# lazear/sage

Hardware: AMD Instinct MI355X
Metric: spectra/sec (whole node), fragment-index search-and-score, human tryptic narrow search (higher is better)
Workload: dtype f32

## Files before the change

### include/sage_hip.h

```cpp
#ifndef SAGE_HIP_H
#define SAGE_HIP_H

#include <stddef.h>
#include <stdint.h>

#ifdef __cplusplus
extern "C" {
#endif

#define SAGE_HIP_ABI_VERSION 6

enum {
    SAGE_HIP_OK = 0,
    SAGE_HIP_ERR_INVALID = 1,
    SAGE_HIP_ERR_NO_DEVICE = 2,
    SAGE_HIP_ERR_HIP = 3,
    SAGE_HIP_ERR_UNSUPPORTED = 4,
    SAGE_HIP_ERR_OOM = 5,
    SAGE_HIP_ERR_INTERNAL = 6
};

enum { SAGE_TOL_PPM = 0, SAGE_TOL_PCT = 1, SAGE_TOL_DA = 2 };
typedef struct SageTolerance {
    int32_t kind;
// ... 160 lines not shown
    uint64_t capacity;
    uint64_t* psm_off;
    uint8_t* kinds;
    int32_t* charges;
    int32_t* fragment_ordinals;
    float* intensities;
    float* mz_calculated;
    float* mz_experimental;
} SageFragments;
int sage_hip_annotate_resident(SageScorer* scorer, SageDeviceBatch* batch, const SageFeature* features,
                               const uint32_t* counts, SageFragments* out);

int sage_hip_quick_score_resident(SageScorer* scorer, SageDeviceBatch* batch, int prefilter_low_memory, uint8_t* keep);

typedef struct SageTiming {
    float prelim_ms;
    float rescore_ms;
    float total_ms;
    uint32_t n_launches;
    uint32_t n_wide;
    uint32_t arena_entries;
    uint32_t n_retry;
    float retry_ms;
    uint32_t n_tied;
    uint32_t n_ways;
} SageTiming;
int sage_hip_last_timing(const SageScorer* scorer, SageTiming* out);
int sage_hip_scorer_set_timing_interval(SageScorer* scorer, uint32_t every);

int sage_hip_host_alloc(uint64_t bytes, void** out);
void sage_hip_host_free(void* p);

int sage_hip_debug_phase_cycles(SageScorer* scorer, unsigned long long* out32);

typedef struct SageRescoreInput {
    uint64_t n;
    const SageFeature* features;
    const float* aligned_rt;
    const float* delta_rt_model;
    const float* delta_ims_model;
    SageTolerance precursor_tol;
    const uint32_t* peptide_key;
    uint32_t n_peptide_keys;
    const uint32_t* protein_key;
    uint32_t n_protein_keys;
} SageRescoreInput;

typedef struct SageRescoreOutput {
    float* discriminant_score;
    float* posterior_error;
    float* spectrum_q;
    float* peptide_q;
    float* protein_q;
    uint32_t* order;
    uint64_t passing_spectrum;
    uint64_t passing_peptide;
    uint64_t passing_protein;
    int32_t lda_fitted;
    double coef[20];
    float device_ms;
} SageRescoreOutput;

int sage_hip_rescore(int device, const SageRescoreInput* in, SageRescoreOutput* out);

typedef struct SageRtInput {
    uint64_t n;
// ... 168 lines not shown
```

### sage_amd/_lib.py

```python
import ctypes as C
import os

import numpy as np

from . import build as _build

c_float_p = C.POINTER(C.c_float)
c_u8_p = C.POINTER(C.c_uint8)
c_u32_p = C.POINTER(C.c_uint32)
c_u64_p = C.POINTER(C.c_uint64)


class SageTolerance(C.Structure):
    _fields_ = [("kind", C.c_int32), ("lo", C.c_float), ("hi", C.c_float)]


class SageTheoretical(C.Structure):
    _fields_ = [("peptide_index", C.c_uint32), ("fragment_mz", C.c_float)]


class SageDbParams(C.Structure):
    _fields_ = [
        ("bucket_size", C.c_uint64),
        ("missed_cleavages", C.c_int32),
# ... 241 lines not shown
        "sage_hip_abi_version": (C.c_int, []),
        "sage_hip_hostdb_build": (C.c_int, [C.c_char_p, C.POINTER(SageDbParams), C.POINTER(vp)]),
        "sage_hip_hostdb_free": (None, [vp]),
        "sage_hip_hostdb_view": (C.c_int, [vp, C.POINTER(SageDbView)]),
        "sage_hip_hostdb_peptide_string": (C.c_uint64, [vp, C.c_uint64, C.c_char_p, C.c_uint64]),
        "sage_hip_hostdb_peptide_proteins": (C.c_uint64, [vp, C.c_uint64, C.c_char_p, C.c_uint64]),
        "sage_hip_hostdb_peptide_info": (C.c_int, [vp, C.c_uint64, c_u32_p, c_u8_p]),
        "sage_hip_process_ms2": (C.c_uint64, [C.c_uint64, C.c_int, C.c_float, c_float_p, c_float_p, C.c_uint64,
                                              C.c_uint8, c_float_p, c_float_p, c_float_p]),
        "sage_hip_device_count": (C.c_int, []),
        "sage_hip_db_create": (C.c_int, [C.POINTER(SageDbView), C.c_int, C.POINTER(vp)]),
        "sage_hip_db_destroy": (None, [vp]),
        "sage_hip_db_device_bytes": (C.c_uint64, [vp]),
        "sage_hip_scorer_create": (C.c_int, [vp, C.POINTER(SageScorerParams), C.POINTER(vp)]),
        "sage_hip_scorer_destroy": (None, [vp]),
        "sage_hip_scorer_clone": (C.c_int, [vp, C.POINTER(vp)]),
        "sage_hip_score_batch": (C.c_int, [vp, C.POINTER(SageSpectrumBatch), vp, c_u32_p]),
        "sage_hip_batch_upload": (C.c_int, [vp, C.POINTER(SageSpectrumBatch), C.POINTER(vp)]),
        "sage_hip_batch_free": (None, [vp]),
        "sage_hip_batch_process_upload": (C.c_int, [vp, C.POINTER(SageRawBatch), C.c_uint64, C.c_int, C.c_float, C.c_uint32,
                                                    C.POINTER(vp), c_u32_p]),
        "sage_hip_batch_download": (C.c_int, [vp, c_u64_p, c_float_p, c_float_p, c_float_p]),
        "sage_hip_batch_upload_kinds": (C.c_int, [vp, C.POINTER(SageSpectrumBatch), c_u8_p, C.POINTER(vp)]),
        "sage_hip_batch_process_upload_kinds": (C.c_int, [vp, C.POINTER(SageRawBatch), c_u8_p, C.c_uint64, C.c_int, C.c_float,
                                                          C.c_uint32, C.POINTER(vp), c_u32_p]),
        "sage_hip_score_batch_kinds": (C.c_int, [vp, C.POINTER(SageSpectrumBatch), c_u8_p, vp, c_u32_p]),
        "sage_hip_score_resident": (C.c_int, [vp, vp, vp, c_u32_p]),
        "sage_hip_initial_hits": (C.c_int, [vp, vp, c_u64_p, C.c_uint32, c_u32_p, c_u64_p, c_u64_p]),
        "sage_hip_last_timing": (C.c_int, [vp, C.POINTER(SageTiming)]),
        "sage_hip_scorer_set_timing_interval": (C.c_int, [vp, C.c_uint32]),
        "sage_hip_annotate_resident": (C.c_int, [vp, vp, vp, c_u32_p, C.POINTER(SageFragments)]),
        "sage_hip_quick_score_resident": (C.c_int, [vp, vp, C.c_int, c_u8_p]),
        "sage_hip_debug_phase_cycles": (C.c_int, [vp, c_u64_p]),
        "sage_hip_host_alloc": (C.c_int, [C.c_uint64, C.POINTER(vp)]),
        "sage_hip_host_free": (None, [vp]),
        "sage_hip_rescore": (C.c_int, [C.c_int, C.POINTER(SageRescoreInput), C.POINTER(SageRescoreOutput)]),
        "sage_hip_hostdb_competition_keys": (C.c_int, [vp, c_u32_p, C.c_uint64, c_u32_p, c_u32_p, c_u32_p, c_u32_p]),
        "sage_hip_predict_rt": (C.c_int, [C.c_int, C.POINTER(SageRtInput), C.POINTER(SageRtOutput)]),
        "sage_hip_hostdb_feature_peptides": (C.c_int, [vp, c_u32_p, C.c_uint64, c_u64_p, c_u8_p, c_float_p]),
        "sage_hip_mzml_read": (C.c_int, [C.c_char_p, C.c_uint32, C.c_int, C.POINTER(vp)]),
        "sage_hip_mzml_view": (C.c_int, [vp, C.POINTER(SageRawBatch)]),
        "sage_hip_mzml_check_searchable": (C.c_int, [vp]),
        "sage_hip_mzml_spectrum_id": (C.c_char_p, [vp, C.c_uint64]),
        "sage_hip_mzml_free": (None, [vp]),
        "sage_hip_mzml_read_sn": (C.c_int, [C.c_char_p, C.c_uint32, C.c_int, C.c_int, C.POINTER(vp)]),
        "sage_hip_mzml_ion_injection_time": (C.c_float, [vp, C.c_uint64]),
        "sage_hip_mzml_precursor_ref": (C.c_char_p, [vp, C.c_uint64]),
        "sage_hip_mgf_read": (C.c_int, [C.c_char_p, C.c_uint32, C.POINTER(vp)]),
        "sage_hip_mzml_isolation_kinds": (C.c_int, [vp, c_u8_p]),
        "sage_hip_mzml_charge_zero": (C.c_int, [vp, c_u8_p]),
        "sage_hip_parse_f32": (C.c_int, [C.c_char_p, C.c_uint64, c_float_p]),
        "sage_hip_tmt": (C.c_int, [C.c_int, C.POINTER(SageTmtInput), C.POINTER(SageTmtOutput)]),
        "sage_hip_write_tmt": (C.c_int, [C.c_char_p, C.POINTER(C.c_char_p), C.c_uint32, C.c_uint64, c_u32_p, C.POINTER(C.c_char_p),
                                         c_float_p, c_float_p, C.POINTER(C.c_char_p), C.c_uint32]),
        "sage_hip_write_results": (C.c_int, [C.c_char_p, C.c_int, vp, vp, C.c_uint64, c_u64_p, c_u64_p, C.POINTER(C.c_char_p),
                                             C.c_uint32, C.POINTER(C.c_char_p), C.POINTER(SagePostColumns)]),
        "sage_hip_lfq": (C.c_int, [C.c_int, C.POINTER(SageLfqInput), C.POINTER(SageLfqOutput)]),
        "sage_hip_lfq_im": (C.c_int, [C.c_int, C.POINTER(SageLfqInput), C.POINTER(SageLfqMobility), C.POINTER(SageLfqOutput)]),
        "sage_hip_mzml_mobility": (c_float_p, [vp]),
        "sage_hip_mzml_has_mobility": (C.c_int, [vp, c_u8_p]),
        "sage_hip_write_lfq": (C.c_int, [C.c_char_p, vp, C.POINTER(SageLfqOutput), c_u64_p, C.c_uint64, C.POINTER(C.c_char_p),
                                         C.c_uint32]),
        "sage_hip_fasta_num_targets": (C.c_int, [C.c_char_p, C.POINTER(SageDbParams), c_u64_p]),
        "sage_hip_prefilter_chunk_size": (C.c_int, [C.c_char_p, C.POINTER(SageDbParams), C.c_uint64, c_u64_p]),
        "sage_hip_hostdb_build_chunk": (C.c_int, [C.c_char_p, C.POINTER(SageDbParams), C.c_uint64, C.c_uint64, C.POINTER(vp)]),
        "sage_hip_hostdb_merge_kept": (C.c_int, [C.POINTER(vp), C.POINTER(c_u8_p), C.c_uint32, C.POINTER(SageDbParams),
                                                 C.POINTER(vp)]),
    }
    for name, (res, args) in sig.items():
        fn = getattr(lib, name)
        fn.restype = res
        fn.argtypes = args
    _lib = lib
    return lib


EXPORTED_SYMBOLS = [
    "sage_hip_last_error", "sage_hip_abi_version", "sage_hip_hostdb_build", "sage_hip_hostdb_free",
    "sage_hip_hostdb_view", "sage_hip_hostdb_peptide_string", "sage_hip_hostdb_peptide_proteins",
    "sage_hip_hostdb_peptide_info", "sage_hip_process_ms2", "sage_hip_device_count", "sage_hip_db_create", "sage_hip_db_destroy",
    "sage_hip_db_device_bytes", "sage_hip_scorer_create", "sage_hip_scorer_destroy", "sage_hip_scorer_clone", "sage_hip_score_batch",
    "sage_hip_batch_upload", "sage_hip_batch_free", "sage_hip_batch_process_upload", "sage_hip_batch_download", "sage_hip_score_resident", "sage_hip_initial_hits",
    "sage_hip_last_timing", "sage_hip_scorer_set_timing_interval", "sage_hip_annotate_resident", "sage_hip_quick_score_resident", "sage_hip_debug_phase_cycles", "sage_hip_host_alloc", "sage_hip_host_free",
    "sage_hip_rescore", "sage_hip_hostdb_competition_keys", "sage_hip_fasta_num_targets", "sage_hip_prefilter_chunk_size",
    "sage_hip_hostdb_build_chunk", "sage_hip_hostdb_merge_kept", "sage_hip_predict_rt", "sage_hip_hostdb_feature_peptides",
    "sage_hip_write_results", "sage_hip_mzml_read", "sage_hip_mzml_view", "sage_hip_mzml_check_searchable", "sage_hip_mzml_spectrum_id", "sage_hip_mzml_free",
    "sage_hip_lfq", "sage_hip_write_lfq", "sage_hip_mzml_read_sn", "sage_hip_mzml_ion_injection_time", "sage_hip_mzml_precursor_ref",
    "sage_hip_tmt", "sage_hip_write_tmt", "sage_hip_mgf_read", "sage_hip_mzml_isolation_kinds", "sage_hip_mzml_charge_zero",
    "sage_hip_parse_f32", "sage_hip_batch_upload_kinds", "sage_hip_batch_process_upload_kinds", "sage_hip_score_batch_kinds",
    "sage_hip_lfq_im", "sage_hip_mzml_mobility", "sage_hip_mzml_has_mobility",
]


def check(rc):
    if rc != 0:
        msg = load().sage_hip_last_error()
        raise SageHipError(f"libsage_hip status {rc}: {msg.decode() if msg else ''}")


def as_ptr(arr, ctype):
    return arr.ctypes.data_as(C.POINTER(ctype))
```

### sage_amd/csrc/capi.hip

```cpp
#include <hip/hip_runtime.h>
#include <algorithm>
#include <atomic>
#include <cmath>
#include <chrono>
#include <cstring>
#include <memory>
#include <future>
#include <mutex>
#include <string>
#include <vector>

#include "crlog.h"
#include "device_types.h"
#define HIP_FAILED(e, what) fail(status_of(e), std::string(what) + ": " + hipGetErrorString(e))
#include "hip_host.h"
#include "host_db.hpp"

using namespace sagehip;

namespace {

thread_local std::string g_last_error;

int fail(int code, const std::string& msg) {
// ... 721 lines not shown
            const double a = std::fabs((double)b);
            ok = ok && a > 0.0 && (double)ion_lo / 255.0 * a >= 2.0 * lo && (double)ion_hi * a <= 0.5 * hi;
        }
    if (ok) mode |= sagecore::TOL_FAST;
    return mode;
}

static int scorer_init(SageScorer* sp, SageDeviceDb* db, const SageScorerParams* p) {
    SageScorer* s = sp;
    s->db = db;
    s->params = *p;
    DevScorer& d = s->dev;
    d.precursor_tol = {p->precursor_tol.kind, p->precursor_tol.lo, p->precursor_tol.hi};
    d.fragment_tol = {p->fragment_tol.kind, p->fragment_tol.lo, p->fragment_tol.hi};
    d.pbm_reach = sagecore::pbm_reach_of(d.fragment_tol);
    d.min_matched_peaks = p->min_matched_peaks;
    d.min_isotope_err = p->min_isotope_err;
    d.max_isotope_err = p->max_isotope_err;
    d.min_precursor_charge = p->min_precursor_charge;
    d.max_precursor_charge = p->max_precursor_charge;
    d.override_precursor_charge = p->override_precursor_charge;
    d.max_fragment_charge = p->max_fragment_charge;
    d.chimera = p->chimera;
    d.report_psms = p->report_psms;
    d.wide_window = p->wide_window;
    d.score_type = p->score_type;
    d.kmax = std::max<uint32_t>(50, 2 * p->report_psms);
    const uint32_t n_iso = (uint32_t)(p->max_isotope_err - p->min_isotope_err) + 1;
    const uint32_t n_z = (uint32_t)(p->max_precursor_charge - p->min_precursor_charge) + 1;
    d.list_cap = d.kmax * (std::max(n_iso, n_z) + 1);
    d.wcap = 1024;
    d.dbg_flags = 0;
    if (const char* e = getenv("SAGE_HIP_DEBUG_FLAGS")) d.dbg_flags = (uint32_t)atoi(e);
    d.rescore_general = 0;
    if (const char* e = getenv("SAGE_HIP_RESCORE_GENERAL")) d.rescore_general = atoi(e) != 0 ? 1u : 0u;
    d.exact = 0;
    d.xcd_chunk = 1024;
    if (const char* e = getenv("SAGE_HIP_XCD_CHUNK")) d.xcd_chunk = (uint32_t)std::max(0, atoi(e));
    {
        const char* e = getenv("SAGE_HIP_SCHED_DESC");
        if (!e || atoi(e)) d.xcd_chunk |= 0x80000000u;
        s->sched_desc_forced = e != nullptr;
    }
    if (const char* e = getenv("SAGE_HIP_EXACT")) s->exact_always = atoi(e) != 0;
    if (const char* e = getenv("SAGE_HIP_FUSED")) s->fused = atoi(e) != 0;
    if (const char* e = getenv("SAGE_HIP_ONE_LANE")) s->two_lanes = atoi(e) == 0;
    if (const char* e = getenv("SAGE_HIP_SEARCH_LAG")) s->search_lag = (uint32_t)std::max(0, atoi(e));
    if (const char* e = getenv("SAGE_HIP_REPLAY_WAVE_MAX")) s->replay_split = (uint64_t)atoll(e) & 0xFFFFFFFFull;
    if (const char* e = getenv("SAGE_HIP_REPLAY_LANE_MAX")) s->replay_split |= (uint64_t)(uint32_t)atoll(e) << 32;
    if (const char* e = getenv("SAGE_HIP_ONE_LAUNCH")) s->one_launch = atoi(e) != 0;
#ifndef SAGE_HIP_EXPERIMENTS
    if (s->one_launch || s->fused || getenv("SAGE_HIP_SEARCH_LAG"))
        return fail(SAGE_HIP_ERR_UNSUPPORTED, "SAGE_HIP_ONE_LAUNCH / SAGE_HIP_FUSED / SAGE_HIP_SEARCH_LAG need a build with -DSAGE_HIP_EXPERIMENTS");
#endif
    if (const char* e = getenv("SAGE_HIP_NO_ZEROCOPY")) s->zero_copy = atoi(e) == 0;
    if (const char* e = getenv("SAGE_HIP_NO_FAST_TIES")) s->fast_ties = atoi(e) == 0;
    if (const char* e = getenv("SAGE_HIP_WCAP")) d.wcap = (uint32_t)std::min(16384, std::max(64, atoi(e)));
    if (const char* e = getenv("SAGE_HIP_CHUNK")) s->chunk = (uint32_t)std::min(1 << 22, std::max(64, atoi(e)));
    HIP_TRY(hipStreamCreateWithFlags(&s->stream, hipStreamNonBlocking));
    HIP_TRY(hipStreamCreateWithFlags(&s->up_stream, hipStreamNonBlocking));
    HIP_TRY(hipStreamCreateWithFlags(&s->down_stream, hipStreamNonBlocking));
    HIP_TRY(hipStreamCreateWithFlags(&s->side_stream, hipStreamNonBlocking));
    if (const char* e = getenv("SAGE_HIP_WAYS")) s->ways = (uint32_t)std::min(4, std::max(1, atoi(e)));
    if (p->report_psms != 1 || p->chimera) s->fast_ties = false;
    if ((d.wcap + 1) / 2 > fast_tie_lds_words()) s->fast_ties = false;
    s->cnt_stride = 4u + (((d.wcap + 1) / 2 + 3u) & ~3u);
// ... 21 lines not shown
        HIP_TRY(o.down_done.create(false));
        HIP_TRY(o.counters.alloc(2 * CTR_COUNT));
        HIP_TRY(hipHostMalloc((void**)&o.h_counters, 2 * CTR_COUNT * 4, hipHostMallocDefault));
        HIP_TRY(hipHostGetDevicePointer((void**)&o.h_counters_view, o.h_counters, 0));
    }
    for (SageDeviceBatch& b : s->slots) {
        b.device = db->device;
        HIP_TRY(b.up_done.create(false));
    }
    std::vector<double> tbl(131072);
    tbl[0] = 1.0;
    for (uint32_t n = 1; n < tbl.size(); n++) {
        const double x = (double)n;
        tbl[n] = x * sagecore::cr_log(x) - x + 0.5 * sagecore::cr_log(x) + 0.5 * sagecore::cr_log(M_PI * 2.0 * x);
    }
    HIP_TRY(s->lnfact.upload(tbl.data(), tbl.size()));
    {
        hipDeviceProp_t prop;
        HIP_TRY(hipGetDeviceProperties(&prop, db->device));
        const size_t tile_lds = ((size_t)1 << db->view.tile_shift) * 2 + 12 * 1024;
        const uint32_t per_cu = (uint32_t)std::max<size_t>(1, std::min<size_t>(4, (160 * 1024) / tile_lds));
        s->tile_blocks = (uint32_t)prop.multiProcessorCount * per_cu;
        const size_t tile_lds8 = ((size_t)1 << db->view.tile_shift) + 14 * 1024;
        s->tile_blocks8 = (uint32_t)prop.multiProcessorCount * (uint32_t)std::max<size_t>(1, std::min<size_t>(4, (160 * 1024) / tile_lds8));
        if (const char* e = getenv("SAGE_HIP_TILE_BLOCKS")) s->tile_blocks = s->tile_blocks8 = (uint32_t)std::max(1, atoi(e));
        if (const char* e = getenv("SAGE_HIP_NO_U8")) s->cnt8 = atoi(e) == 0;
        if (const char* e = getenv("SAGE_HIP_NO_REUSE")) s->reuse_counts = atoi(e) == 0;
        HIP_TRY((hipError_t)tile_kernel_prepare(160 * 1024));
        HIP_TRY((hipError_t)spectrum_kernel_prepare(160 * 1024));
    }
    s->qmax = queries_per_spectrum(d);
    if (const char* e = getenv("SAGE_HIP_PHASE_CLOCKS")) {
        if (atoi(e) > 0) {
            HIP_TRY(s->dbg.alloc(4096 * 32));
            HIP_TRY(hipMemset(s->dbg.p, 0, 4096 * 32 * 8));
        }
    }
    return SAGE_HIP_OK;
}

static void scorer_release(SageScorer* s) {
    (void)hipSetDevice(s->db->device);
    for (hipStream_t st : {s->stream, s->up_stream, s->down_stream, s->side_stream, s->way_stream[0], s->way_stream[1], s->way_stream[2]})
        if (st) {
            (void)hipStreamSynchronize(st);
            (void)hipStreamDestroy(st);
        }
    delete s;
}

int sage_hip_scorer_create(SageDeviceDb* db, const SageScorerParams* p, SageScorer** out) {
    if (!db || !p || !out) return fail(SAGE_HIP_ERR_INVALID, "null argument");
    if (p->report_psms == 0) return fail(SAGE_HIP_ERR_INVALID, "report_psms must be >= 1");
    if (p->report_psms > 32767) return fail(SAGE_HIP_ERR_UNSUPPORTED, "report_psms > 32767");
    if (p->min_isotope_err > p->max_isotope_err) return fail(SAGE_HIP_ERR_INVALID, "min_isotope_err > max_isotope_err");
    if (p->min_precursor_charge > p->max_precursor_charge || p->min_precursor_charge == 0)
        return fail(SAGE_HIP_ERR_INVALID, "precursor charge range must be [lo >= 1, hi >= lo]");
    if (p->score_type != 0 && p->score_type != 1) return fail(SAGE_HIP_ERR_INVALID, "unknown score_type");
    HIP_TRY(hipSetDevice(db->device));
    SageScorer* s = new SageScorer();
    const int rc = scorer_init(s, db, p);
    if (rc != SAGE_HIP_OK) {
        s->db = db;
        scorer_release(s);
        return rc;
    }
    *out = s;
    return SAGE_HIP_OK;
// ... 1136 lines not shown
    int rc = enqueue_compute(s, b->view, o, false, MODE_EXACT, s->stream);
    if (rc != SAGE_HIP_OK) return rc;
    HIP_TRY(hipMemcpyAsync(o.h_counters, o.counters.p, 2 * CTR_COUNT * 4, hipMemcpyDeviceToHost, s->stream));
    HIP_TRY(hipStreamSynchronize(s->stream));
    rc = collect(s, o, nullptr);
    if (rc != SAGE_HIP_OK) return rc;
    const uint32_t n = b->n, kmax = s->dev.kmax;
    std::vector<uint64_t> c((size_t)n * kmax);
    std::vector<uint32_t> tot((size_t)n * 2), st(n);
    HIP_TRY(hipMemcpy(c.data(), s->ws.cand.p, c.size() * 8, hipMemcpyDeviceToHost));
    HIP_TRY(hipMemcpy(len, s->ws.cand_len.p, (size_t)n * 4, hipMemcpyDeviceToHost));
    HIP_TRY(hipMemcpy(tot.data(), s->ws.totals.p, tot.size() * 4, hipMemcpyDeviceToHost));
    HIP_TRY(hipMemcpy(st.data(), s->ws.status.p, (size_t)n * 4, hipMemcpyDeviceToHost));
    for (uint32_t i = 0; i < n; i++) {
        if (st[i] != ST_OK && st[i] != ST_OK_ORDERED) return fail(SAGE_HIP_ERR_UNSUPPORTED, "spectrum " + std::to_string(i) + ": status " + std::to_string(st[i]));
        for (uint32_t j = 0; j < len[i]; j++) packed[(size_t)i * cap + j] = c[(size_t)i * kmax + j];
        if (matched_peaks) matched_peaks[i] = tot[2 * i];
        if (scored_candidates) scored_candidates[i] = tot[2 * i + 1];
    }
    return SAGE_HIP_OK;
}

int sage_hip_debug_phase_cycles(SageScorer* s, unsigned long long* out32) {
    if (!s || !out32) return fail(SAGE_HIP_ERR_INVALID, "null argument");
    if (!s->dbg.p) return fail(SAGE_HIP_ERR_INVALID, "set SAGE_HIP_PHASE_CLOCKS=1 before creating the scorer");
    std::vector<unsigned long long> all(4096 * 32);
    HIP_TRY(hipMemcpy(all.data(), s->dbg.p, all.size() * 8, hipMemcpyDeviceToHost));
    for (int k = 0; k < 32; k++) out32[k] = 0;
    for (size_t b = 0; b < 4096; b++)
        for (int k = 0; k < 32; k++) out32[k] += all[b * 32 + k];
    return SAGE_HIP_OK;
}

int sage_hip_host_alloc(uint64_t bytes, void** out) {
    if (!out) return fail(SAGE_HIP_ERR_INVALID, "null argument");
    HIP_TRY(hipHostMalloc(out, bytes ? bytes : 1, hipHostMallocDefault));
    if (void* d = device_view(*out)) {
        std::lock_guard<std::mutex> lock(g_blocks_mu);
        g_blocks.push_back(HostBlock{(const unsigned char*)*out, (unsigned char*)d, (size_t)(bytes ? bytes : 1)});
    }
    return SAGE_HIP_OK;
}
void sage_hip_host_free(void* p) {
    if (!p) return;
    {
        std::lock_guard<std::mutex> lock(g_blocks_mu);
        for (size_t i = 0; i < g_blocks.size(); i++)
            if (g_blocks[i].host == (const unsigned char*)p) {
                g_blocks.erase(g_blocks.begin() + (long)i);
                break;
            }
    }
    (void)hipHostFree(p);
}

int sage_hip_scorer_set_timing_interval(SageScorer* s, uint32_t every) {
    if (!s) return fail(SAGE_HIP_ERR_INVALID, "null argument");
    std::lock_guard<std::mutex> lock(s->mu);
    s->timing_every = every;
    s->timing_calls = 0;
    return SAGE_HIP_OK;
}

int sage_hip_last_timing(const SageScorer* s, SageTiming* out) {
    if (!s || !out) return fail(SAGE_HIP_ERR_INVALID, "null argument");
    *out = s->timing;
// ... 25 lines not shown
```

### sage_amd/csrc/device_types.h

```cpp
#pragma once
#include <stdint.h>

#include <string>

#include "../../include/sage_hip.h"
#include "core.h"

namespace sagehip {

struct DevDbView {
    const float* pep_mono;
    uint32_t np;
    const uint32_t* pep_lut;
    uint32_t pep_lut_bins;
    float pep_lut_inv_w;
    const SageTheoretical* pm_frag;
    const uint64_t* pm_off;
    const float* ions;
    const uint64_t* ion_off;
    const uint32_t* pep_info;
    const SageTheoretical* tm_frag;
    const uint32_t* tm_lut;
    uint32_t tile_shift;
    uint32_t n_tiles;
    uint32_t lut_stride;
    float lut_scale;
    const SageTheoretical* tm2_frag;
    const sagecore::LutWord* tm2_l1;
    const uint32_t* tm2_pos;
    uint32_t lut2_words;
    uint32_t tile2_shift;
    uint32_t n_tiles2;
    uint32_t lut2_stride;
    float lut2_scale;
    uint64_t nf;
    uint8_t ion_kinds[8];
    uint32_t n_kinds;
};

#ifndef SAGE_TM_LUT_TRANSPOSED
#define SAGE_TM_LUT_TRANSPOSED 0
#endif
#ifndef SAGE_TM_LUT_QUAD
#define SAGE_TM_LUT_QUAD 0
#endif
constexpr int TM_LUT_LAYOUT = SAGE_TM_LUT_QUAD != 0 ? 2 : SAGE_TM_LUT_TRANSPOSED != 0 ? 1 : 0;
constexpr bool TM_LUT_TRANSPOSED = TM_LUT_LAYOUT == 1;
__host__ __device__ inline uint32_t tm_lut_rows(uint32_t n_tiles) { return TM_LUT_LAYOUT == 2 ? (n_tiles + 3u) & ~3u : n_tiles; }
__host__ __device__ inline size_t tm_lut_index(uint32_t t, uint32_t c, uint32_t n_tiles, uint32_t lut_stride) {
    return TM_LUT_LAYOUT == 2 ? (((size_t)(t >> 2) * lut_stride + c) << 2) + (t & 3u)
           : TM_LUT_LAYOUT == 1 ? (size_t)c * n_tiles + t : (size_t)t * lut_stride + c;
}

struct DevScorer {
    sagecore::Tol precursor_tol, fragment_tol;
    sagecore::PbmReach pbm_reach;
    uint32_t min_matched_peaks;
    int min_isotope_err, max_isotope_err;
    uint32_t min_precursor_charge, max_precursor_charge;
    uint32_t override_precursor_charge;
    int max_fragment_charge;
    uint32_t chimera;
    uint32_t report_psms;
    uint32_t wide_window;
    int score_type;
    uint32_t kmax;
    uint32_t big_path;
    uint32_t long_runs;
    uint32_t tol_mode;
    uint32_t list_cap;
    uint32_t wcap;
    uint32_t dbg_flags;
    uint32_t rescore_general;
    uint32_t xcd_chunk;
    uint32_t fast_log;
    uint32_t exact;
};

struct DevBatchView {
    uint32_t n;
    const uint32_t* n_dev;
    uint32_t spec_base;
    const uint64_t* peak_off;
    const float* masses;
    const float* intensities;
    const float* precursor_mz;
    const uint8_t* precursor_charge;
    const float* isolation_lo;
    const float* isolation_hi;
    const float* tic;
    const float* rt;
    const float* ims;
    const uint32_t* file_id;
    const uint32_t* order;
    uint32_t probe;
    uint32_t pcap;
    uint32_t fzcap;
    const uint4* sched;
    const uint8_t* iso_kind;
};

struct DevWork {
    uint64_t* cand;
    uint32_t* cand_len;
    uint32_t* totals;
// ... 138 lines not shown
```

### sage_amd/csrc/kernels.hip

```cpp
#include <hip/hip_runtime.h>

#include <type_traits>

#include "crlog.h"
#include "device_types.h"

using namespace sagecore;

namespace sagehip {

namespace {

constexpr uint32_t WAVE = 64;
constexpr uint32_t FAST_TIE_WORDS = PBM_WORDS + PLUT_BINS;
constexpr uint32_t CNT_ROW_HEADER = 4;
#ifndef SAGE_PROBE_PER_LANE
#define SAGE_PROBE_PER_LANE 2
#endif
constexpr uint32_t PROBE_BATCH_WORDS = SAGE_PROBE_PER_LANE * 64;
constexpr uint32_t PROBE_TCS_WORDS = PROBE_BATCH_WORDS <= 64 ? 64 : PROBE_BATCH_WORDS <= 128 ? 128 : PROBE_BATCH_WORDS <= 256 ? 256 : 512;
constexpr uint32_t PROBE_TABLE_WORDS = 4 * PROBE_BATCH_WORDS + PROBE_TCS_WORDS;

constexpr uint32_t DBG_BLOCKS = 4096;
enum { DBG_NARROW_LUT = 26, DBG_NARROW_CELLS = 27, DBG_RESCORE = 28, DBG_TILE_LUT = 29, DBG_TILE_CELLS = 30, DBG_TILE_CAND = 31 };
struct PhaseClock {
    unsigned long long* slot;
    long long t;
    __device__ __forceinline__ void bytes(int which, unsigned long long n) {
        if (slot) atomicAdd(&slot[which - row_base], n);
    }
    int row_base;
    __device__ __forceinline__ void start(unsigned long long* dbg, uint32_t blk, uint32_t kernel) {
        slot = dbg ? dbg + (size_t)(blk % DBG_BLOCKS) * 32 + kernel * 8 : nullptr;
        row_base = (int)kernel * 8;
        if (slot) t = clock64();
    }
    __device__ __forceinline__ void mark(int phase) {
        if (slot) {
            const long long n = clock64();
            if ((threadIdx.x & 63u) == 0) atomicAdd(&slot[phase], (unsigned long long)(n - t));
            t = n;
        }
    }
    __device__ __forceinline__ void rebase(uint32_t kernel) {
        if (slot) slot += (int)kernel * 8 - row_base;
        row_base = (int)kernel * 8;
    }
};

struct NoClock {
    static constexpr unsigned long long* slot = nullptr;
    __device__ __forceinline__ void bytes(int, unsigned long long) {}
    __device__ __forceinline__ void start(unsigned long long*, uint32_t, uint32_t) {}
    __device__ __forceinline__ void mark(int) {}
    __device__ __forceinline__ void rebase(uint32_t) {}
};

__device__ __forceinline__ uint32_t lane_id() { return threadIdx.x & 63u; }

#ifndef SAGE_STAGGER_NS
#define SAGE_STAGGER_NS 0
#endif
__device__ __forceinline__ void staggered_start(uint32_t blk) {
    if (SAGE_STAGGER_NS > 0 && blk >= 1024u && blk < 5u * 1024u) {
        const uint32_t slot = blk / 1024u;
        const long long until = (long long)__builtin_amdgcn_s_memtime() + (long long)slot * (SAGE_STAGGER_NS * 2);
        while ((long long)__builtin_amdgcn_s_memtime() < until) __builtin_amdgcn_s_sleep(32);
    }
}

constexpr uint32_t N_XCD = 8;
__device__ __forceinline__ uint32_t xcd_position_fwd(uint32_t b, uint32_t n, uint32_t chunk) {
    if (chunk == 0) return b;
    const uint32_t group = N_XCD * chunk;
    if (b >= n / group * group) return b;
    const uint32_t x = b % N_XCD, i = b / N_XCD;
    return ((i / chunk) * N_XCD + x) * chunk + i % chunk;
}
__device__ __forceinline__ uint32_t xcd_position(uint32_t b, uint32_t n, uint32_t chunk) {
    const uint32_t p = xcd_position_fwd(b, n, chunk & 0x7FFFFFFFu);
    return (chunk & 0x80000000u) ? n - 1 - p : p;
}

__device__ __forceinline__ uint32_t fresh_zero() {
    uint32_t z;
// ... 2518 lines not shown
    const uint32_t nions = scored ? db.n_kinds * lm1 : 0u;
    for (uint32_t j0 = 0; __ballot(j0 < nions) != 0ull; j0 += 64u) {
        const bool act = j0 < nions;
        const uint32_t n_here = !act ? 0u : nions - j0 < 64u ? nions - j0 : 64u;
        uint64_t m1 = 0, m2 = 0, m3 = 0;
        if (act) {
            const float* __restrict__ q = my + j0;
            float n0, n1, n2, n3;
            if (have_first && j0 == 0) { n0 = first0; n1 = first1; n2 = first2; n3 = first3; }
            else { n0 = q[0]; n1 = q[1]; n2 = q[2]; n3 = q[3]; }
            for (uint32_t r = 0; r < n_here; r += 4) {
                const float i0 = n0, i1 = n1, i2 = n2, i3 = n3;
                n0 = q[r + 4]; n1 = q[r + 5]; n2 = q[r + 6]; n3 = q[r + 7];
                const uint32_t x0 = pbm_index(i0), x1 = pbm_index(i1), x2 = pbm_index(i2), x3 = pbm_index(i3);
                const uint32_t t1 = pbm_bit(x0) | (pbm_bit(x1) << 1) | (pbm_bit(x2) << 2) | (pbm_bit(x3) << 3);
                m1 |= (uint64_t)t1 << r;
                if (any_fz2) {
                    const uint32_t t2 = pbm_bit(x0 >> 1) | (pbm_bit(x1 >> 1) << 1) | (pbm_bit(x2 >> 1) << 2) | (pbm_bit(x3 >> 1) << 3);
                    m2 |= (uint64_t)t2 << r;
                }
                if (any_fz3) {
                    const uint32_t t3 = pbm_bit(__umulhi(x0, 0xAAAAAAABu) >> 1) | (pbm_bit(__umulhi(x1, 0xAAAAAAABu) >> 1) << 1) |
                                        (pbm_bit(__umulhi(x2, 0xAAAAAAABu) >> 1) << 2) | (pbm_bit(__umulhi(x3, 0xAAAAAAABu) >> 1) << 3);
                    m3 |= (uint64_t)t3 << r;
                }
            }
            const uint64_t in_chunk = n_here >= 64u ? ~0ull : (1ull << n_here) - 1ull;
            m1 &= in_chunk;
            m2 = nfz >= 2 ? m2 & in_chunk : 0ull;
            m3 = nfz >= 3 ? m3 & in_chunk : 0ull;
            if (nfz > 3) m1 = m2 = m3 = in_chunk;
        }
        pc.mark(6);
        const uint32_t hc = act && nfz <= 3 ? (uint32_t)(__popcll(m1) + __popcll(m2) + __popcll(m3)) : 0u;
        uint64_t bigs = (sc.dbg_flags & 32u) ? 0ull : __ballot(hc > COOP_MIN_HITS);
        if ((uint32_t)__popcll(bigs) > COOP_MAX_LANES && !(sc.dbg_flags & 64u)) bigs = 0ull;
        while (bigs) {
            const uint32_t L = (uint32_t)__ffsll((long long)bigs) - 1;
            bigs &= bigs - 1;
            const uint64_t M1 = lane_value(m1, L), M2 = lane_value(m2, L), M3 = lane_value(m3, L);
            const uint64_t base_L = lane_value((uint64_t)ion_base, L);
            const uint32_t lm1_L = (uint32_t)__builtin_amdgcn_readlane((int)lm1, (int)L);
            const bool on1 = (M1 >> lane) & 1ull, on2 = (M2 >> lane) & 1ull, on3 = (M3 >> lane) & 1ull;
            float it1 = 0.f, it2 = 0.f, it3 = 0.f, tm1 = 0.f, tm2 = 0.f, tm3 = 0.f;
            bool ok1 = false, ok2 = false, ok3 = false;
            if (on1 || on2 || on3) {
                const float ionv = db.ions[base_L + j0 + lane];
#define SAGE_COOP_LOOKUP(C, ON, OK, IT, TM)                                                              \
    if (ON) {                                                                                            \
        const float mz = fragment_mz<FAST>(ionv, (C));                                                   \
        float flo, fhi;                                                                                  \
        tol_bounds_mode<FAST>(sc.fragment_tol, sym_tol, mz, flo, fhi);                                   \
        const int pk = select_peak_lut(pm, pi, P, plut, inv_w, flo, fhi);                                \
        if (pk >= 0) {                                                                                   \
const float peak_mass = pm[pk], peak_intensity = pi[pk];                                     \
OK = true;                                                                                   \
IT = peak_intensity;                                                                         \
TM = peak_intensity * __builtin_fabsf(mz - peak_mass) * 2E6f / (mz + peak_mass);             \
        }                                                                                                \
    }
                SAGE_COOP_LOOKUP(1, on1, ok1, it1, tm1)
                SAGE_COOP_LOOKUP(2, on2, ok2, it2, tm2)
                SAGE_COOP_LOOKUP(3, on3, ok3, it3, tm3)
#undef SAGE_COOP_LOOKUP
            }
            const uint64_t K1 = __ballot(ok1), K2 = __ballot(ok2), K3 = __ballot(ok3);
            float u_sb = lane_valuef(s.summed_b, L), u_sy = lane_valuef(s.summed_y, L), u_pp = lane_valuef(s.ppm_difference, L);
// ... 186 lines not shown
    for (int q = 0; q < 6; q++) f.pad[q] = 0;
    return f;
}

struct RescoreKernargs {
    DevDbView db;
    DevScorer sc;
    DevBatchView b;
    DevWork w;
    const double* lnfact_table;
    uint32_t lnfact_n;
    SageFeature* out;
    uint32_t* out_count;
    uint8_t* keep;
};
template <class K>
struct LateArgs {
    const DevDbView& db;
    const DevScorer& sc;
    const DevBatchView& b;
    const DevWork& w;
    const double* lnfact_table_;
    uint32_t lnfact_n_;
    SageFeature* out_;
    uint32_t* out_count_;
    __device__ __forceinline__ LateArgs(const DevDbView& db_, const DevScorer& sc_, const DevBatchView& b_, const DevWork& w_, const double* t,
                                        uint32_t tn, SageFeature* o, uint32_t* oc)
        : db(db_), sc(sc_), b(b_), w(w_), lnfact_table_(t), lnfact_n_(tn), out_(o), out_count_(oc) {}
    __device__ __forceinline__ void refresh() {}
    __device__ __forceinline__ const float* ions() const { return db.ions; }
    __device__ __forceinline__ uint32_t report_psms() const { return sc.report_psms; }
    __device__ __forceinline__ uint32_t chimera() const { return sc.chimera; }
    __device__ __forceinline__ uint32_t min_matched_peaks() const { return sc.min_matched_peaks; }
    __device__ __forceinline__ int score_type() const { return sc.score_type; }
    __device__ __forceinline__ uint32_t xcd_chunk() const { return sc.xcd_chunk; }
    __device__ __forceinline__ uint32_t batch_n() const { return b.n; }
    __device__ __forceinline__ uint32_t spec_base() const { return b.spec_base; }
    __device__ __forceinline__ uint32_t* status() const { return w.status; }
    __device__ __forceinline__ uint32_t* retry() const { return w.retry; }
    __device__ __forceinline__ uint32_t* counters() const { return w.n_deferred; }
    __device__ __forceinline__ const uint32_t* cnt_store() const { return w.cnt_store; }
    __device__ __forceinline__ uint32_t cnt_stride() const { return w.cnt_stride; }
    __device__ __forceinline__ const double* lnfact_table() const { return lnfact_table_; }
    __device__ __forceinline__ uint32_t lnfact_n() const { return lnfact_n_; }
    __device__ __forceinline__ SageFeature* out() const { return out_; }
    __device__ __forceinline__ uint32_t* out_count() const { return out_count_; }
    __device__ __forceinline__ uint8_t* keep(uint8_t* k) const { return k; }
};
template <>
struct LateArgs<RescoreKernargs> {
    typedef const __attribute__((address_space(4))) RescoreKernargs* Segment;
    Segment ka;
    __device__ __forceinline__ LateArgs(const DevDbView&, const DevScorer&, const DevBatchView&, const DevWork&, const double*, uint32_t, SageFeature*,
                                        uint32_t*)
        : ka((Segment)__builtin_amdgcn_kernarg_segment_ptr()) {}
    __device__ __forceinline__ void refresh() {
        ka = (Segment)__builtin_amdgcn_kernarg_segment_ptr();
        asm volatile("" : "+s"(ka));
    }
    __device__ __forceinline__ const float* ions() const { return ka->db.ions; }
    __device__ __forceinline__ uint32_t report_psms() const { return ka->sc.report_psms; }
    __device__ __forceinline__ uint32_t chimera() const { return ka->sc.chimera; }
    __device__ __forceinline__ uint32_t min_matched_peaks() const { return ka->sc.min_matched_peaks; }
    __device__ __forceinline__ int score_type() const { return ka->sc.score_type; }
    __device__ __forceinline__ uint32_t xcd_chunk() const { return ka->sc.xcd_chunk; }
    __device__ __forceinline__ uint32_t batch_n() const { return ka->b.n; }
    __device__ __forceinline__ uint32_t spec_base() const { return ka->b.spec_base; }
    __device__ __forceinline__ uint32_t* status() const { return ka->w.status; }
    __device__ __forceinline__ uint32_t* retry() const { return ka->w.retry; }
    __device__ __forceinline__ uint32_t* counters() const { return ka->w.n_deferred; }
    __device__ __forceinline__ const uint32_t* cnt_store() const { return ka->w.cnt_store; }
    __device__ __forceinline__ uint32_t cnt_stride() const { return ka->w.cnt_stride; }
    __device__ __forceinline__ const double* lnfact_table() const { return ka->lnfact_table; }
    __device__ __forceinline__ uint32_t lnfact_n() const { return ka->lnfact_n; }
    __device__ __forceinline__ SageFeature* out() const { return ka->out; }
    __device__ __forceinline__ uint32_t* out_count() const { return ka->out_count; }
    __device__ __forceinline__ uint8_t* keep(uint8_t*) const { return ka->keep; }
};

template <bool ACC, class KA, bool FAST = false, bool CHIMERA = true, class PC>
__device__ __forceinline__ bool rescore_spectrum(const DevDbView& db, const DevScorer& sc, const DevBatchView& b, const DevWork& w,
                                                 const double* __restrict__ lnfact_table, uint32_t lnfact_n,
                                                 SageFeature* __restrict__ out, uint32_t* __restrict__ out_count,
                                                 uint8_t* __restrict__ keep, const RescoreLds& R, const uint32_t spec, uint32_t P,
                                                 const uint64_t mine, const uint32_t tot_matched, const uint32_t tot_scored,
                                                 const bool list_is_exact, const bool queue_on_tie, PC& pc) {
    const uint32_t lane = lane_id();
    uint32_t* const pbm = R.pbm;
    uint32_t* const plut = R.plut;
    float* const pm = R.pm;
    float* const pi = R.pi;
    const uint32_t pep = prescore_peptide(mine);
    const bool valid = pep != 0xFFFFFFFFu;
    const uint32_t z = prescore_charge(mine);
    const int iso = prescore_iso(mine);
    const uint32_t nfz = max_fragment_charge(sc.max_fragment_charge, z) - 1;
// ... 38 lines not shown
            if (SAGE_ION_PREFETCH && lm1 && nfz) {
                const float* __restrict__ q = db.ions + ion_base;
                first0 = q[0]; first1 = q[1]; first2 = q[2]; first3 = q[3];
            }
        }
        if (round == 0) build_peak_bitmap(pbm, pm, P, sc.pbm_reach);
        lds_sync();
        if (round == 0) {
        if (pc.slot) {
            const uint32_t ion_bytes = wave_sum(valid ? 4u * db.n_kinds * lm1 + 24u : 0u);
            const uint32_t ncand = (uint32_t)__popcll(__ballot(mine != PRESCORE_EMPTY));
            if (lane == 0) pc.bytes(DBG_RESCORE, 8ull * P + 8ull * ncand + ion_bytes);
            const uint32_t items = wave_sum(SAGE_N_ITEMS);
            uint32_t longest = SAGE_N_ITEMS;
            for (int o = 32; o; o >>= 1) { const uint32_t v = (uint32_t)__shfl_xor((int)longest, o, 64); longest = v > longest ? v : longest; }
            const uint32_t nvalid = (uint32_t)__popcll(__ballot(valid));
            (void)items; (void)longest; (void)nvalid;
        }
        }
        Score s;
        s.peptide = 0;
        s.precursor_charge = 0;
        s.isotope_error = 0;
        s.matched_b = s.matched_y = 0;
        s.summed_b = s.summed_y = 0.0f;
        s.ppm_difference = 0.0f;
        s.longest_b = s.longest_y = 0;
        pc.mark(5);
        score_candidates<PC, false, FAST>(db, sc, pbm, plut, pm, pi, P, inv_w, valid, ion_base, lm1, nfz, any_fz2, any_fz3, nterm_mask, sym_tol,
                                          s, pc, SAGE_ION_PREFETCH && round == 0, first0, first1, first2, first3, !CHIMERA || !sc.chimera);
        pc.mark(1);
        LateArgs<KA> la(db, sc, b, w, lnfact_table, lnfact_n, out, out_count);
        la.refresh();
        const double lambda = (double)R.hdr[HDR_MATCHED] / (double)R.hdr[HDR_SCORED];
        double h = 0.0;
        bool pass = false;
        bool ln_undecided;
        const double ln_i = cr_log_pair<ACC>(hyperscore_arg(s), lambda, round == 0, ((__ballot(valid) >> 63) & 1ull) == 0ull, ln_lambda, ln_undecided);
        if (__builtin_expect(!ACC && __ballot(ln_undecided && (valid || round == 0)) != 0ull, 0)) {
            if (queue_on_tie && lane == 0) {
                la.status()[spec] = ST_RETRY;
                la.retry()[atomicAdd(la.counters() + CTR_RETRY, 1u)] = spec;
                la.out_count()[spec] = 0;
            }
            return false;
        }
        if (valid) {
            s.ppm_difference /= s.summed_b + s.summed_y;
            h = hyperscore_dev(la.score_type(), s, ln_i, la.lnfact_table(), la.lnfact_n());
            pass = (s.matched_b + s.matched_y) >= la.min_matched_peaks();
        }
        const uint32_t report_psms = la.report_psms();
        const bool chimera = CHIMERA && la.chimera() != 0u;
        const uint32_t per_round = chimera ? 1u : report_psms;
        if (ACC && keep) {
            QuickKey* qk = R.qkeys;
            QuickKey mk;
            mk.peptide = pep; mk.matched_b = s.matched_b; mk.matched_y = s.matched_y;
            mk.summed_b = s.summed_b; mk.summed_y = s.summed_y; mk.longest_b = s.longest_b; mk.longest_y = s.longest_y;
            mk.hyperscore = h; mk.ppm_difference = s.ppm_difference; mk.charge = z; mk.iso = iso;
            qk[lane] = mk;
            const uint64_t pmask = __ballot(pass);
            const uint32_t npass = (uint32_t)__popcll(pmask);
            const uint32_t kq = report_psms < npass ? report_psms : npass;
            __syncthreads();
            if (pass) {
// ... 930 lines not shown
```

Measured before the change: 135.0 million.

## Prune candidates that cannot reach min matched peaks before scoring

During candidate tiling, a lane's hits are dropped on its last ion chunk when the accumulated matched count plus the current hits still falls below min_matched_peaks. That removes cooperative scoring work for candidates that could never pass. In rescore, if no lane in the wave can meet the threshold, the spectrum skips the log-probability and hyperscore computation and leaves early. Debug counters for pruning statistics and a flag to disable pruning are added too; correctness depends on the count-based bound being exact.

```diff
diff --git a/include/sage_hip.h b/include/sage_hip.h
--- a/include/sage_hip.h
+++ b/include/sage_hip.h
@@ -216,6 +216,7 @@
 void sage_hip_host_free(void* p);
 
 int sage_hip_debug_phase_cycles(SageScorer* scorer, unsigned long long* out32);
+int sage_hip_debug_prune_counters(SageScorer* scorer, unsigned long long* out4);
 
 typedef struct SageRescoreInput {
     uint64_t n;
diff --git a/sage_amd/_lib.py b/sage_amd/_lib.py
--- a/sage_amd/_lib.py
+++ b/sage_amd/_lib.py
@@ -297,6 +297,7 @@
         "sage_hip_annotate_resident": (C.c_int, [vp, vp, vp, c_u32_p, C.POINTER(SageFragments)]),
         "sage_hip_quick_score_resident": (C.c_int, [vp, vp, C.c_int, c_u8_p]),
         "sage_hip_debug_phase_cycles": (C.c_int, [vp, c_u64_p]),
+        "sage_hip_debug_prune_counters": (C.c_int, [vp, c_u64_p]),
         "sage_hip_host_alloc": (C.c_int, [C.c_uint64, C.POINTER(vp)]),
         "sage_hip_host_free": (None, [vp]),
         "sage_hip_rescore": (C.c_int, [C.c_int, C.POINTER(SageRescoreInput), C.POINTER(SageRescoreOutput)]),
@@ -346,7 +347,7 @@
     "sage_hip_hostdb_peptide_info", "sage_hip_process_ms2", "sage_hip_device_count", "sage_hip_db_create", "sage_hip_db_destroy",
     "sage_hip_db_device_bytes", "sage_hip_scorer_create", "sage_hip_scorer_destroy", "sage_hip_scorer_clone", "sage_hip_score_batch",
     "sage_hip_batch_upload", "sage_hip_batch_free", "sage_hip_batch_process_upload", "sage_hip_batch_download", "sage_hip_score_resident", "sage_hip_initial_hits",
-    "sage_hip_last_timing", "sage_hip_scorer_set_timing_interval", "sage_hip_annotate_resident", "sage_hip_quick_score_resident", "sage_hip_debug_phase_cycles", "sage_hip_host_alloc", "sage_hip_host_free",
+    "sage_hip_last_timing", "sage_hip_scorer_set_timing_interval", "sage_hip_annotate_resident", "sage_hip_quick_score_resident", "sage_hip_debug_phase_cycles", "sage_hip_debug_prune_counters", "sage_hip_host_alloc", "sage_hip_host_free",
     "sage_hip_rescore", "sage_hip_hostdb_competition_keys", "sage_hip_fasta_num_targets", "sage_hip_prefilter_chunk_size",
     "sage_hip_hostdb_build_chunk", "sage_hip_hostdb_merge_kept", "sage_hip_predict_rt", "sage_hip_hostdb_feature_peptides",
     "sage_hip_write_results", "sage_hip_mzml_read", "sage_hip_mzml_view", "sage_hip_mzml_check_searchable", "sage_hip_mzml_spectrum_id", "sage_hip_mzml_free",
diff --git a/sage_amd/csrc/capi.hip b/sage_amd/csrc/capi.hip
--- a/sage_amd/csrc/capi.hip
+++ b/sage_amd/csrc/capi.hip
@@ -777,6 +777,7 @@
     d.wcap = 1024;
     d.dbg_flags = 0;
     if (const char* e = getenv("SAGE_HIP_DEBUG_FLAGS")) d.dbg_flags = (uint32_t)atoi(e);
+    d.prune_min = (d.dbg_flags & 4096u) ? 0u : d.min_matched_peaks;
     d.rescore_general = 0;
     if (const char* e = getenv("SAGE_HIP_RESCORE_GENERAL")) d.rescore_general = atoi(e) != 0 ? 1u : 0u;
     d.exact = 0;
@@ -864,8 +865,8 @@
     s->qmax = queries_per_spectrum(d);
     if (const char* e = getenv("SAGE_HIP_PHASE_CLOCKS")) {
         if (atoi(e) > 0) {
-            HIP_TRY(s->dbg.alloc(4096 * 32));
-            HIP_TRY(hipMemset(s->dbg.p, 0, 4096 * 32 * 8));
+            HIP_TRY(s->dbg.alloc(DBG_TOTAL_WORDS));
+            HIP_TRY(hipMemset(s->dbg.p, 0, DBG_TOTAL_WORDS * 8));
         }
     }
     return SAGE_HIP_OK;
@@ -2068,6 +2069,17 @@
     return SAGE_HIP_OK;
 }
 
+int sage_hip_debug_prune_counters(SageScorer* s, unsigned long long* out4) {
+    if (!s || !out4) return fail(SAGE_HIP_ERR_INVALID, "null argument");
+    if (!s->dbg.p) return fail(SAGE_HIP_ERR_INVALID, "set SAGE_HIP_PHASE_CLOCKS=1 before creating the scorer");
+    std::vector<unsigned long long> all((size_t)DBG_BLOCKS * DBG_PRUNE_WORDS);
+    HIP_TRY(hipMemcpy(all.data(), s->dbg.p + (size_t)DBG_BLOCKS * 32, all.size() * 8, hipMemcpyDeviceToHost));
+    for (uint32_t k = 0; k < DBG_PRUNE_WORDS; k++) out4[k] = 0;
+    for (size_t b = 0; b < DBG_BLOCKS; b++)
+        for (uint32_t k = 0; k < DBG_PRUNE_WORDS; k++) out4[k] += all[b * DBG_PRUNE_WORDS + k];
+    return SAGE_HIP_OK;
+}
+
 int sage_hip_host_alloc(uint64_t bytes, void** out) {
     if (!out) return fail(SAGE_HIP_ERR_INVALID, "null argument");
     HIP_TRY(hipHostMalloc(out, bytes ? bytes : 1, hipHostMallocDefault));
diff --git a/sage_amd/csrc/device_types.h b/sage_amd/csrc/device_types.h
--- a/sage_amd/csrc/device_types.h
+++ b/sage_amd/csrc/device_types.h
@@ -52,6 +52,9 @@
            : TM_LUT_LAYOUT == 1 ? (size_t)c * n_tiles + t : (size_t)t * lut_stride + c;
 }
 
+constexpr uint32_t DBG_BLOCKS = 4096, DBG_PRUNE_WORDS = 4;
+constexpr size_t DBG_TOTAL_WORDS = (size_t)DBG_BLOCKS * (32 + DBG_PRUNE_WORDS);
+
 struct DevScorer {
     sagecore::Tol precursor_tol, fragment_tol;
     sagecore::PbmReach pbm_reach;
@@ -71,6 +74,7 @@
     uint32_t list_cap;
     uint32_t wcap;
     uint32_t dbg_flags;
+    uint32_t prune_min;
     uint32_t rescore_general;
     uint32_t xcd_chunk;
     uint32_t fast_log;
diff --git a/sage_amd/csrc/kernels.hip b/sage_amd/csrc/kernels.hip
--- a/sage_amd/csrc/kernels.hip
+++ b/sage_amd/csrc/kernels.hip
@@ -21,7 +21,7 @@
 constexpr uint32_t PROBE_TCS_WORDS = PROBE_BATCH_WORDS <= 64 ? 64 : PROBE_BATCH_WORDS <= 128 ? 128 : PROBE_BATCH_WORDS <= 256 ? 256 : 512;
 constexpr uint32_t PROBE_TABLE_WORDS = 4 * PROBE_BATCH_WORDS + PROBE_TCS_WORDS;
 
-constexpr uint32_t DBG_BLOCKS = 4096;
+enum { DBG_PRUNE_CAND = 0, DBG_PRUNE_ITEMS = 1, DBG_PRUNE_EARLY = 2, DBG_PRUNE_MIXED = 3 };
 enum { DBG_NARROW_LUT = 26, DBG_NARROW_CELLS = 27, DBG_RESCORE = 28, DBG_TILE_LUT = 29, DBG_TILE_CELLS = 30, DBG_TILE_CAND = 31 };
 struct PhaseClock {
     unsigned long long* slot;
@@ -30,9 +30,29 @@
         if (slot) atomicAdd(&slot[which - row_base], n);
     }
     int row_base;
+    unsigned long long* prune;
+    uint32_t pruned_here;
+    __device__ __forceinline__ void pruned(uint64_t lanes, uint32_t items) {
+        if (slot && lanes) {
+            pruned_here += (uint32_t)__popcll(lanes);
+            if ((threadIdx.x & 63u) == 0) {
+                atomicAdd(&prune[DBG_PRUNE_CAND], (unsigned long long)__popcll(lanes));
+                atomicAdd(&prune[DBG_PRUNE_ITEMS], (unsigned long long)items);
+            }
+        }
+    }
+    __device__ __forceinline__ void prune_outcome(bool left_early, bool any_pass) {
+        if (slot && (threadIdx.x & 63u) == 0) {
+            if (left_early) atomicAdd(&prune[DBG_PRUNE_EARLY], 1ull);
+            else if (any_pass && pruned_here) atomicAdd(&prune[DBG_PRUNE_MIXED], 1ull);
+        }
+        pruned_here = 0;
+    }
     __device__ __forceinline__ void start(unsigned long long* dbg, uint32_t blk, uint32_t kernel) {
         slot = dbg ? dbg + (size_t)(blk % DBG_BLOCKS) * 32 + kernel * 8 : nullptr;
         row_base = (int)kernel * 8;
+        prune = dbg ? dbg + (size_t)DBG_BLOCKS * 32 + (size_t)(blk % DBG_BLOCKS) * DBG_PRUNE_WORDS : nullptr;
+        pruned_here = 0;
         if (slot) t = clock64();
     }
     __device__ __forceinline__ void mark(int phase) {
@@ -51,6 +71,8 @@
 struct NoClock {
     static constexpr unsigned long long* slot = nullptr;
     __device__ __forceinline__ void bytes(int, unsigned long long) {}
+    __device__ __forceinline__ void pruned(uint64_t, uint32_t) {}
+    __device__ __forceinline__ void prune_outcome(bool, bool) {}
     __device__ __forceinline__ void start(unsigned long long*, uint32_t, uint32_t) {}
     __device__ __forceinline__ void mark(int) {}
     __device__ __forceinline__ void rebase(uint32_t) {}
@@ -2635,7 +2657,15 @@
             if (nfz > 3) m1 = m2 = m3 = in_chunk;
         }
         pc.mark(6);
-        const uint32_t hc = act && nfz <= 3 ? (uint32_t)(__popcll(m1) + __popcll(m2) + __popcll(m3)) : 0u;
+        uint32_t hc = act && nfz <= 3 ? (uint32_t)(__popcll(m1) + __popcll(m2) + __popcll(m3)) : 0u;
+        {
+            const bool drop = hc != 0u && j0 + 64u >= nions && (mm & 0xFFFFu) + (mm >> 16) + hc < sc.prune_min;
+            if (pc.slot) pc.pruned(__ballot(drop), wave_sum(drop ? hc : 0u));
+            if (drop) {
+                m1 = m2 = m3 = 0ull;
+                hc = 0u;
+            }
+        }
         uint64_t bigs = (sc.dbg_flags & 32u) ? 0ull : __ballot(hc > COOP_MIN_HITS);
         if ((uint32_t)__popcll(bigs) > COOP_MAX_LANES && !(sc.dbg_flags & 64u)) bigs = 0ull;
         while (bigs) {
@@ -2888,6 +2918,7 @@
     __device__ __forceinline__ uint32_t report_psms() const { return sc.report_psms; }
     __device__ __forceinline__ uint32_t chimera() const { return sc.chimera; }
     __device__ __forceinline__ uint32_t min_matched_peaks() const { return sc.min_matched_peaks; }
+    __device__ __forceinline__ uint32_t prune_min() const { return sc.prune_min; }
     __device__ __forceinline__ int score_type() const { return sc.score_type; }
     __device__ __forceinline__ uint32_t xcd_chunk() const { return sc.xcd_chunk; }
     __device__ __forceinline__ uint32_t batch_n() const { return b.n; }
@@ -2918,6 +2949,7 @@
     __device__ __forceinline__ uint32_t report_psms() const { return ka->sc.report_psms; }
     __device__ __forceinline__ uint32_t chimera() const { return ka->sc.chimera; }
     __device__ __forceinline__ uint32_t min_matched_peaks() const { return ka->sc.min_matched_peaks; }
+    __device__ __forceinline__ uint32_t prune_min() const { return ka->sc.prune_min; }
     __device__ __forceinline__ int score_type() const { return ka->sc.score_type; }
     __device__ __forceinline__ uint32_t xcd_chunk() const { return ka->sc.xcd_chunk; }
     __device__ __forceinline__ uint32_t batch_n() const { return ka->b.n; }
@@ -3022,6 +3054,16 @@
         pc.mark(1);
         LateArgs<KA> la(db, sc, b, w, lnfact_table, lnfact_n, out, out_count);
         la.refresh();
+        {
+            const uint32_t prune_min = la.prune_min();
+            const uint64_t can_pass = __ballot(valid && s.matched_b + s.matched_y >= prune_min);
+            const bool leave = prune_min != 0u && can_pass == 0ull;
+            pc.prune_outcome(leave, can_pass != 0ull);
+            if (leave) {
+                if (ACC && keep) return true;
+                break;
+            }
+        }
         const double lambda = (double)R.hdr[HDR_MATCHED] / (double)R.hdr[HDR_SCORED];
         double h = 0.0;
         bool pass = false;
```

Measured after the change: 138.4 million (median of 6 runs). 2.5% higher.
